# chhylp123/hifiasm

Measured on AMD Instinct MI355X. Metric: read-pair overlaps/sec (sum ol->length / (ha_pt_gen + all-reads h_ec_lchain pass)), higher is better.
Workload: dtype u64 hashing / int32 + f64 chain scores

## Files before the change

### hifiasm_amd/csrc/hao_chain.cuh

```cuda
#pragma once
#include "hao_common.cuh"
#include "hao_host.hpp"
#include "hao_query.cuh"

#define HAO_MCOPY_MAX 3

struct hao_chain_rec {
	uint32_t x_pos_s, x_pos_e, y_pos_s, y_pos_e; int32_t score; uint32_t n_hits, hit_rel, fc_rel, fc_len, strand;
	uint32_t src_rel, in_place;
};

#define HH_ID(h)     ((h).w0 & 0x7fffffffu)
#define HH_STRAND(h) ((h).w0 >> 31)
#define HH_SPAN(h)   ((int32_t)((h).cnt & 0xffu))
#define HH_WGT(h)    ((int32_t)((h).cnt >> 8))

struct hao_cpar { double pen_gap, pen_skip, bw; int64_t max_skip, max_iter, max_dis, xl, yl; };

__device__ __forceinline__ int64_t hao_ext_len(int64_t x_beg, int64_t x_end, int64_t xl, int64_t y_beg, int64_t y_end, int64_t yl)
{
	if (x_beg <= y_beg) x_beg = 0; else x_beg -= y_beg;
	int64_t xr = xl - x_end - 1, yr = yl - y_end - 1;
	if (xr <= yr) x_end = xl - 1; else x_end += yr;
	return x_end - x_beg + 1;
}

__device__ __forceinline__ int32_t hao_band(const hao_hit_t &ai, const hao_hit_t &aj, const hao_cpar &P)
{
	int64_t sf_s = aj.self_offset, sf_e = (int64_t)ai.self_offset + 1, ot_s = aj.offset, ot_e = (int64_t)ai.offset + 1;
	int64_t sf_r = P.xl - sf_e, ot_r = P.yl - ot_e;
	if (sf_s <= ot_s) sf_s = 0; else sf_s -= ot_s;
	if (sf_r <= ot_r) sf_e = P.xl; else sf_e += ot_r;
	return (int32_t)((double)(sf_e - sf_s) * P.bw);
}

__device__ __forceinline__ int32_t hao_pair_score(const hao_hit_t &ai, const hao_hit_t &aj, const hao_cpar &P, int64_t *dd_out)
{
	int32_t dq = (int32_t)((int64_t)ai.self_offset - (int64_t)aj.self_offset); if (dq <= 0) return INT32_MIN;
	int32_t dr = (int32_t)((int64_t)ai.offset - (int64_t)aj.offset); if (dr <= 0) return INT32_MIN;
	int32_t dd = dr > dq ? dr - dq : dq - dr;
	if (dd > 16 && dd > hao_band(ai, aj, P)) return INT32_MIN;
	int32_t dg = dr < dq ? dr : dq, span = HH_SPAN(ai), sc = span < dg ? span : dg, wgt = HH_WGT(ai);
	if (wgt != 1) sc = sc >= wgt ? (wgt == 2 ? sc >> 1 : sc / wgt) : 1;
	if (dd) {
		double lin = P.pen_gap * (double)dd; const double skip = P.pen_skip * (double)dg;
		if (!(dd < 4 && lin + skip < 1.0)) {
			const double ap = (double)sc * (((double)dd / (double)dg) / P.bw);
			if (dd < 4) lin = lin > ap ? ap : lin; else lin = lin < ap ? ap : lin;
			lin += skip;
			sc -= (int32_t)lin;
		}
	} else if (dg > span) {
		sc -= (int32_t)(0.0 + P.pen_skip * (double)dg);
	}
	if (dd_out) *dd_out = dd;
	return sc;
}

__device__ __forceinline__ void hao_region(hao_chain_rec &o, int64_t xl, int64_t yl, int64_t sc, const hao_hit_t &beg, const hao_hit_t &end)
{
	o.strand = HH_STRAND(beg);
	o.x_pos_s = beg.self_offset; o.y_pos_s = beg.offset; o.x_pos_e = end.self_offset; o.y_pos_e = end.offset;
	if (o.x_pos_s <= o.y_pos_s) { o.y_pos_s -= o.x_pos_s; o.x_pos_s = 0; } else { o.x_pos_s -= o.y_pos_s; o.y_pos_s = 0; }
	int64_t xr = xl - o.x_pos_e - 1, yr = yl - o.y_pos_e - 1;
	if (xr <= yr) { o.x_pos_e = (uint32_t)(xl - 1); o.y_pos_e += (uint32_t)xr; } else { o.y_pos_e = (uint32_t)(yl - 1); o.x_pos_e += (uint32_t)yr; }
	o.score = (int32_t)sc;
}

__device__ __forceinline__ uint64_t hao_fc_entry(uint32_t site, int32_t shift)
{ uint32_t lo = shift < 0 ? ((uint32_t)(-shift) << 1 | 1u) : (uint32_t)shift << 1; return (uint64_t)site << 32 | lo; }

template<class HitAt>
__device__ uint32_t hao_fake_cigar(uint64_t *fc, const hao_chain_rec &o, HitAt hit, int64_t n_hit)
{
	int64_t pdd = INT32_MAX; uint32_t n = 0;
	fc[n++] = hao_fc_entry(o.x_pos_s, 0);
	for (int64_t k = 0; k < n_hit; ++k) {
		const hao_hit_t h = hit(k);
		int64_t dq = (int64_t)h.self_offset - o.x_pos_s, dr = (int64_t)h.offset - o.y_pos_s, dd = dr - dq;
		if (dd != pdd) { pdd = dd; fc[n++] = hao_fc_entry(h.self_offset, (int32_t)pdd); }
	}
	uint64_t last = fc[n - 1]; int32_t lsh = (int32_t)((uint32_t)last >> 1); if (last & 1) lsh = -lsh;
	if ((int64_t)(int32_t)(last >> 32) != (int64_t)o.x_pos_e) fc[n++] = hao_fc_entry(o.x_pos_e, lsh);
	return n;
}

// ... 104 lines not shown
						hao_region(rec[n_u], P.xl, P.yl, sc + plus, a[ii[n_v - 1]], a[ii[n_v0]]);
						c_nv0[n_u] = (uint32_t)n_v0; c_ni[n_u] = (uint32_t)(n_v - n_v0); ++n_u;
					} else n_v = n_v0;
				} else n_v = n_v0;
			}
			for (k = 0, i = 0; k < n_u; ++k) {
				n_v0 = c_nv0[k]; ni = c_ni[k];
				rec[k].hit_rel = (uint32_t)i; rec[k].n_hits = (uint32_t)ni; rec[k].src_rel = (uint32_t)i; rec[k].in_place = 0;
				if (A.hcode) hao_code_chain_lane(A, gs, a, i, ni, [&](int64_t q_) { return (int64_t)ii[n_v0 + (ni - q_ - 1)]; });
				for (j = 0; j < ni; ++j, ++i) des[i] = a[ii[n_v0 + (ni - j - 1)]];
				rec[k].fc_rel = fcn; rec[k].fc_len = hao_fake_cigar(fcs + fcn, rec[k], [&](int64_t q_) { return a[ii[n_v0 + (ni - q_ - 1)]]; }, ni); fcn += rec[k].fc_len;
			}
			A.nch[g] = (uint32_t)n_u; A.nout[g] = (uint32_t)i;
			return;
		} else {
			msc += plus; i = msc_i; cL = 0;
			while (i >= 0) { t[cL++] = i; i = p[i]; }
		}
	}
	hao_region(rec[0], P.xl, P.yl, msc, a[t[cL - 1]], a[t[0]]);
	if (A.hcode) hao_code_chain_lane(A, gs, a, 0, cL, [&](int64_t q_) { return (int64_t)t[cL - q_ - 1]; });
	for (i = 0; i < cL; ++i) des[i] = a[t[cL - i - 1]];
	rec[0].hit_rel = 0; rec[0].n_hits = (uint32_t)cL; rec[0].src_rel = 0; rec[0].in_place = 0; rec[0].fc_rel = 0; rec[0].fc_len = hao_fake_cigar(fcs, rec[0], [&](int64_t q_) { return a[t[cL - q_ - 1]]; }, cL);
	A.nch[g] = 1; A.nout[g] = (uint32_t)cL;
}


template<class HitP, class I32P, class I64P>
__device__ void hao_chain_generic_core(const hao_chain_args &A, const uint64_t g, const uint64_t gs, HitP a, const int64_t a_n, const uint32_t xid, const uint32_t yid,
		const uint32_t xl, const uint32_t yl, I32P f, I32P ii, I32P p, I64P t)
{
	A.nch[g] = 0; A.nout[g] = 0;
	if (yid == xid || a_n <= 0) return;
	hao_cpar P; P.pen_gap = A.par.pen_gap; P.pen_skip = A.par.pen_skip; P.bw = A.par.bw; P.max_skip = A.par.max_skip; P.max_iter = A.par.max_iter; P.max_dis = A.par.max_dis;
	P.xl = xl; P.yl = yl;
	int64_t plus = 0, msc = INT32_MIN, msc_i = INT32_MIN, movl = INT32_MAX, si = 0, ei = a_n;
	{
		int64_t l = 0, k, z; bool sorted = true;
		for (k = 1; k <= a_n; ++k) {
			t[k - 1] = 0; ii[k - 1] = 0;
			if (k < a_n && HH_STRAND(a[k]) == HH_STRAND(a[l])) {
				if (a[k].self_offset <= a[k - 1].self_offset || a[k].offset <= a[k - 1].offset) sorted = false;
				continue;
			}
			if (sorted) {
				int64_t plus0 = 0, msc0 = INT32_MIN, msc_i0 = INT32_MIN, ddt = 0, sc, dd = 0;
				p[l] = -1; f[l] = HH_SPAN(a[l]);
				if (f[l] >= msc0) { msc0 = f[l]; msc_i0 = l; }
				if (f[l] < plus0) plus0 = f[l];
				for (z = l + 1; z < k; ++z) {
					int32_t s = hao_pair_score(a[z], a[z - 1], P, &dd);
					if (s == INT32_MIN) break;
					sc = (int64_t)s + f[z - 1];
					if (sc < HH_SPAN(a[z])) break;
					p[z] = (int32_t)(z - 1); f[z] = (int32_t)sc; ddt += dd;
					if (f[z] >= msc0) { msc0 = f[z]; msc_i0 = z; }
					if (f[z] < plus0) plus0 = f[z];
				}
				if (z >= k && msc_i0 == k - 1) {
					if (k - l >= 2 && ddt > 16 && ddt > hao_band(a[k - 1], a[l], P)) msc_i0 = INT32_MIN;
					if (msc_i0 == k - 1) {
						if (msc0 >= msc) {
							int64_t ov = hao_ext_len(a[msc_i0].self_offset, a[msc_i0].self_offset, P.xl, a[msc_i0].offset, a[msc_i0].offset, P.yl);
							if (msc0 > msc || ov < movl) { msc = msc0; msc_i = msc_i0; movl = ov; }
						}
						if (plus0 < plus) plus = plus0;
						if (ei > k) si = k; else ei = l;
// ... 63 lines not shown
			for (int k = 0; k < HAO_TINY_MAX; ++k) if ((uint32_t)k < e.n) l_a[k * 64 + threadIdx.x] = src[k];
		}
		const hao_lane_arr<int32_t> f{l_f + threadIdx.x}, ii{l_ii + threadIdx.x}, p{l_p + threadIdx.x}; const hao_lane_arr<int64_t> t{l_t + threadIdx.x};
		hao_chain_generic_core(A, e.g, e.start, hao_lane_hits{l_a + threadIdx.x}, (int64_t)e.n, (uint32_t)(A.rid_lo + e.r), e.yid, e.xl, e.yl, f, ii, p, t);
	}
}

__device__ __forceinline__ hao_hit_t hao_shfl_hit(const hao_hit_t &h, int src)
{ hao_hit_t o; o.w0 = hao_bcast(h.w0, src); o.offset = hao_bcast(h.offset, src); o.self_offset = hao_bcast(h.self_offset, src); o.cnt = hao_bcast(h.cnt, src); return o; }
__device__ __forceinline__ hao_hit_t hao_shfl_up_hit(const hao_hit_t &h)
{ hao_hit_t o; o.w0 = hao_wave_shr1(h.w0, h.w0); o.offset = hao_wave_shr1(h.offset, h.offset); o.self_offset = hao_wave_shr1(h.self_offset, h.self_offset); o.cnt = hao_wave_shr1(h.cnt, h.cnt); return o; }

__global__ __launch_bounds__(64) __attribute__((amdgpu_num_sgpr(96))) void chain_group_kernel(hao_chain_args A, const hao_gent *list, uint64_t n_list, uint32_t *slow, int cls)
{
	const uint64_t li = blockIdx.x;
	if (li >= n_list) return;
	const int lane = hao_lane();
	__shared__ uint64_t l_eb[2][64];
	uint64_t (*eb)[64] = l_eb; uint32_t ce0 = 0, ce1 = 0;
	const unsigned long long tq0 = A.dbg_qc ? wall_clock64() : 0;
	const hao_gent e = list[li];
	const uint64_t g = e.g, gs = e.start; const int32_t a_n = (int32_t)e.n;
	const hao_hit_t *a = A.hits + gs;
	const uint32_t xid = (uint32_t)(A.rid_lo + e.r), yid = e.yid;
	if (yid == xid || a_n <= 0) {
		if (A.hcode) for (int32_t i = lane; i < a_n; i += 64) A.hcode[gs + i] = 0x08;
		if (lane == 0) { A.nch[g] = 0; A.nout[g] = 0; }
		return;
	}
	hao_hit_t hn = a[lane < a_n ? lane : 0];
	const uint16_t *hqg = A.hcode ? A.hq + gs : nullptr; uint8_t *hcg = A.hcode ? A.hcode + gs : nullptr;
	uint32_t qn = hcg ? hqg[lane < a_n ? lane : 0] : 0u, carry_q = 0;
	const hao_hit_t first0 = hao_shfl_hit(hn, 0);
	hao_cpar P; P.pen_gap = A.par.pen_gap; P.pen_skip = A.par.pen_skip; P.bw = A.par.bw; P.max_skip = A.par.max_skip; P.max_iter = A.par.max_iter; P.max_dis = A.par.max_dis;
	P.xl = e.xl; P.yl = e.yl;
	const unsigned long long tq1 = A.dbg_qc ? wall_clock64() + (first0.w0 & 0) : 0;
	int32_t carry_f = 0; hao_hit_t carry_h = first0; carry_h.w0 ^= 0x80000000u;
	bool fail0 = false, fail1 = false, seen = false; int32_t maxf0 = INT32_MIN, maxf1 = INT32_MIN, flast0 = 0, flast1 = 0, k1 = 0, n_bnd = 0;
	uint32_t ddt0 = 0, ddt1 = 0;
	uint32_t last0_so = first0.self_offset, last0_of = first0.offset, last1_so = last0_so, last1_of = last0_of;
	unsigned long long first = 1ULL;
	const uint32_t ulane = (uint32_t)lane;
	for (int32_t t0 = 0; t0 < a_n; t0 += 64) {
		const int32_t left = a_n - t0; const bool act = lane < left;
		const unsigned long long actm = left >= 64 ? ~0ULL : (1ULL << left) - 1ULL;
		const hao_hit_t h = hn;
		const uint32_t q = qn;
		if (left > 64) {
			const uint32_t j = min(ulane, (uint32_t)(left - 65)); const hao_hit_t *an = a + (t0 + 64);
			hn = an[j]; if (hcg) qn = (hqg + (t0 + 64))[j];
		}
		hao_hit_t ph; ph.w0 = hao_wave_shr1(h.w0, carry_h.w0); ph.offset = hao_wave_shr1(h.offset, carry_h.offset); ph.self_offset = hao_wave_shr1(h.self_offset, carry_h.self_offset); ph.cnt = 0;
		const bool bnd = (int32_t)(h.w0 ^ ph.w0) < 0, st = act && bnd;
		const unsigned long long Mst = __ballot(bnd) & actm, Mbnd = Mst & ~first;
		unsigned long long Mb = 0; uint32_t bthr = 64; int B = 0;
		if (seen) { Mb = actm; bthr = 0; }
		else if (Mbnd) { B = __ffsll((long long)Mbnd) - 1; Mb = (~0ULL << B) & actm; bthr = (uint32_t)B; }
		const int b = ulane >= bthr;
		if (hcg) {
			const int32_t idx = t0 + lane;
			const uint32_t pq = hao_wave_shr1(q, carry_q);
			const int32_t dq = (int32_t)(q - pq), sh = (int32_t)((h.offset - ph.offset) - (h.self_offset - ph.self_offset));
			bool exc = false;
			if (A.exc_every) { uint32_t ii = (uint32_t)idx, ee = A.exc_every; HAO_OPAQUE_U32(ii); HAO_OPAQUE_U32(ee); exc = ii % ee == ee - 1; }
			const uint8_t code = st ? (uint8_t)0x08 : ((dq < 1 || dq > 15 || sh < -8 || sh > 7 || q == 65535u || exc) ? (uint8_t)0xff : (uint8_t)((dq - 1) << 4 | (sh + 8)));
			if (act) hcg[idx] = code;
			carry_q = hao_bcast(q, 63);
		}
		const int32_t span = HH_SPAN(h);
		const int32_t dq = (int32_t)(h.self_offset - ph.self_offset), dr = (int32_t)(h.offset - ph.offset);
		bool bad = dq <= 0 || dr <= 0;
		const int32_t dd = dr > dq ? dr - dq : dq - dr, dg = dr < dq ? dr : dq;
		if (!bad && dd > 16) { if (dd > hao_band(h, ph, P)) bad = true; }
		int32_t sc = span < dg ? span : dg;
		{	const int32_t wgt = HH_WGT(h);
			if (wgt != 1) sc = sc >= wgt ? (wgt == 2 ? sc >> 1 : sc / wgt) : 1; }
		if (dd) {
			double lin = P.pen_gap * (double)dd; const double skip = P.pen_skip * (double)dg;
			if (!(dd < 4 && lin + skip < 1.0)) {
				const double ap = (double)sc * (((double)dd / (double)dg) / P.bw);
				if (dd < 4) lin = lin > ap ? ap : lin; else lin = lin < ap ? ap : lin;
				lin += skip;
				sc -= (int32_t)lin;
			}
		} else if (dg > span) sc -= (int32_t)(0.0 + P.pen_skip * (double)dg);
		const bool scored = act && !bnd && !bad;
		const int32_t s = bad ? INT32_MIN : sc;
		const int32_t x = st ? span : (scored ? sc : 0);
		const uint32_t dde = scored ? (uint32_t)dd : 0u;
		{	const bool cf = act && (bnd || dr != dq);
			const unsigned long long Mcf = (__ballot(dr != dq) | Mst) & actm;
			const uint32_t n0 = (uint32_t)__popcll(Mcf & ~Mb), n1 = (uint32_t)__popcll(Mcf & Mb);
			if (cf) { const uint32_t at = hao_mbcnt(Mcf) + (b ? ce1 - n0 : ce0); if (at < 64) eb[b][at] = (uint64_t)h.self_offset << 32 | (h.offset - h.self_offset); }
			ce0 += n0; ce1 += n1; }
		const int32_t F = (int32_t)hao_wave_incl_scan_u32((uint32_t)x);
		int32_t f;
		if (Mbnd) {
			n_bnd += __popcll(Mbnd);
			const int32_t sub = B ? hao_bcast(F, B - 1) : 0;
			f = lane >= B ? F - sub : F + carry_f;
			if (B) { flast0 = hao_bcast(f, B - 1); last0_so = hao_bcast(h.self_offset, B - 1); last0_of = hao_bcast(h.offset, B - 1); }
			else { flast0 = carry_f; last0_so = carry_h.self_offset; last0_of = carry_h.offset; }
		} else f = F + carry_f;
		const int32_t fp = hao_wave_shr1(f, carry_f);
		const unsigned long long Mbrk = __ballot(hao_add_sat_i32(s, fp) < span) & actm & ~Mst;
		if (Mbrk & ~Mb) fail0 = true;
		if (Mbrk & Mb) fail1 = true;
		if (bthr == 64) { maxf0 = max(maxf0, f); ddt0 = hao_add_sat_u32(ddt0, dde); }
		else if (bthr == 0) { maxf1 = max(maxf1, f); ddt1 = hao_add_sat_u32(ddt1, dde); }
		else if (b == 0) { maxf0 = max(maxf0, f); ddt0 = hao_add_sat_u32(ddt0, dde); } else { maxf1 = max(maxf1, f); ddt1 = hao_add_sat_u32(ddt1, dde); }
		k1 += __popcll(actm & ~Mb);
		if (left <= 64) {
			const int Ls = left - 1; const int32_t vf = hao_bcast(f, Ls); const uint32_t vso = hao_bcast(h.self_offset, Ls), vof = hao_bcast(h.offset, Ls);
			if ((Mb >> Ls) & 1ULL) { flast1 = vf; last1_so = vso; last1_of = vof; } else { flast0 = vf; last0_so = vso; last0_of = vof; }
		}
		carry_f = hao_bcast(f, 63); carry_h = hao_shfl_hit(h, 63);
		if (Mbnd) seen = true;
		first = 0;
// ... 29 lines not shown
	hao_region(rc, P.xl, P.yl, msc, best ? first1 : first0, best ? last1 : last0);
	uint32_t cnt; const uint32_t ce = best ? ce1 : ce0;
	if (ce <= 64) {
		HAO_WAVE_FENCE();
		const int64_t cdiag = (int64_t)rc.y_pos_s - (int64_t)rc.x_pos_s;
		if (lane == 0) fcs[0] = hao_fc_entry(rc.x_pos_s, 0);
		if ((uint32_t)lane < ce) { const uint64_t raw = eb[best][lane]; fcs[1 + lane] = hao_fc_entry((uint32_t)(raw >> 32), (int32_t)((int64_t)(int32_t)(uint32_t)raw - cdiag)); }
		const uint64_t rlast = eb[best][ce - 1];
		cnt = 1 + ce;
		if ((uint32_t)(rlast >> 32) != rc.x_pos_e) { if (lane == 0) fcs[cnt] = hao_fc_entry(rc.x_pos_e, (int32_t)((int64_t)(int32_t)(uint32_t)rlast - cdiag)); ++cnt; }
	} else cnt = hao_fake_cigar_wave(fcs, rc.x_pos_s, rc.y_pos_s, rc.x_pos_e, cL, [&](int64_t k) { return a[bl + k]; });
	if (lane == 0) {
		rc.hit_rel = 0; rc.n_hits = (uint32_t)cL; rc.src_rel = (uint32_t)bl; rc.in_place = 1; rc.fc_rel = 0; rc.fc_len = cnt;
		A.rec[g * HAO_MCOPY_MAX] = rc; A.nch[g] = 1; A.nout[g] = (uint32_t)cL;
		if (A.dbg_qc && (li & 63) == 0) {  const unsigned long long tq3 = wall_clock64(); atomicAdd(A.dbg_qc, tq1 - tq0); atomicAdd(A.dbg_qc + 1, tq2 - tq1); atomicAdd(A.dbg_qc + 2, tq3 - tq2); atomicAdd(A.dbg_qc + 3, 1ULL); atomicAdd(A.dbg_qc + 4, (unsigned long long)a_n); }
	}
}


__global__ __launch_bounds__(256) void chain_pack8_kernel(hao_chain_args A, const hao_gent *list, uint64_t n_list, uint32_t *slow)
{
	const int lane = hao_lane(), wv = threadIdx.x >> 6, seg = lane >> 3, idx = lane & 7, sb = lane & ~7;
	const uint64_t li = ((uint64_t)blockIdx.x * 4 + wv) * 8 + seg;
	const bool have = li < n_list;
	hao_gent e; e.g = 0; e.r = 0; e.start = 0; e.n = 0; e.yid = 0; e.xl = 0; e.yl = 0;
	if (have) e = list[li];
	const int32_t a_n = (int32_t)e.n; const uint64_t g = e.g, gs = e.start;
	const uint32_t xid = (uint32_t)(A.rid_lo + e.r), yid = e.yid;
	const bool skip = !have || yid == xid || a_n <= 0;
	const bool act = !skip && idx < a_n;
	hao_hit_t h; h.w0 = 0; h.offset = 0; h.self_offset = 0; h.cnt = 0;
	if (act) h = A.hits[gs + idx];
	const uint32_t q = (A.hcode && act) ? A.hq[gs + idx] : 0u;
	hao_cpar P; P.pen_gap = A.par.pen_gap; P.pen_skip = A.par.pen_skip; P.bw = A.par.bw; P.max_skip = A.par.max_skip; P.max_iter = A.par.max_iter; P.max_dis = A.par.max_dis;
	P.xl = e.xl; P.yl = e.yl;
	const hao_hit_t ph = hao_shfl_up_hit(h);
	const uint32_t strand0 = (uint32_t)__shfl((int)HH_STRAND(h), sb);
	const bool st = act && (idx == 0 || HH_STRAND(h) != HH_STRAND(ph));
	const int b = act && HH_STRAND(h) != strand0;
	int32_t s = HH_SPAN(h); bool ok = true; int64_t dd = 0;
	if (act && !st) { s = hao_pair_score(h, ph, P, &dd); ok = s != INT32_MIN; if (!ok) { s = 0; dd = 0; } }
	uint8_t code = 0x08;
	if (A.hcode) {
		const uint32_t pq = hao_wave_shr1(q, 0u);
		const int32_t dq = (int32_t)(q - pq), sh = (int32_t)((h.offset - ph.offset) - (h.self_offset - ph.self_offset));
		if (!st) code = (dq < 1 || dq > 15 || sh < -8 || sh > 7 || q == 65535u || (A.exc_every && (uint32_t)idx % A.exc_every == A.exc_every - 1)) ? (uint8_t)0xff : (uint8_t)((dq - 1) << 4 | (sh + 8));
	}
	const uint32_t diag = h.offset - h.self_offset, pdiag = ph.offset - ph.self_offset;
	const bool cf = act && (st || diag != pdiag);
	int32_t x = act ? s : 0; int fl = (st || idx == 0) ? 1 : 0;
	hao_seg_scan_add(x, fl);
	const int32_t f = x, fp = hao_wave_shr1(f, 0);
	const bool brk = act && !st && (!ok || (int64_t)s + fp < (int64_t)HH_SPAN(h));
	auto seg_byte = [&](unsigned long long m) { return (uint32_t)(m >> sb) & 0xffu; };
	const uint32_t in0 = seg_byte(__ballot(act && b == 0)), brk0 = seg_byte(__ballot(brk && b == 0)), brk1 = seg_byte(__ballot(brk && b == 1)),
				   cf0 = seg_byte(__ballot(cf && b == 0)), cf1 = seg_byte(__ballot(cf && b == 1));
	const int32_t k1 = __popc(in0);
	const bool two = k1 < a_n;
	int32_t maxf0 = (act && b == 0) ? f : INT32_MIN, maxf1 = (act && b == 1) ? f : INT32_MIN, ddt0 = (act && b == 0) ? (int32_t)dd : 0, ddt1 = (act && b == 1) ? (int32_t)dd : 0;
#pragma unroll
	for (int d = 1; d < 8; d <<= 1) { maxf0 = max(maxf0, __shfl_xor(maxf0, d)); maxf1 = max(maxf1, __shfl_xor(maxf1, d)); ddt0 += __shfl_xor(ddt0, d); ddt1 += __shfl_xor(ddt1, d); }
	const int l0 = sb + (k1 > 0 ? k1 - 1 : 0), f1 = sb + (two ? k1 : 0), l1 = sb + (a_n > 0 ? a_n - 1 : 0);
	const int32_t flast0 = __shfl(f, l0), flast1 = __shfl(f, l1);
	hao_hit_t first0, last0, first1, last1;
	first0.w0 = (uint32_t)__shfl((int)h.w0, sb); first0.self_offset = (uint32_t)__shfl((int)h.self_offset, sb); first0.offset = (uint32_t)__shfl((int)h.offset, sb); first0.cnt = 0;
	last0.w0 = first0.w0; last0.self_offset = (uint32_t)__shfl((int)h.self_offset, l0); last0.offset = (uint32_t)__shfl((int)h.offset, l0); last0.cnt = 0;
	first1.w0 = (uint32_t)__shfl((int)h.w0, f1); first1.self_offset = (uint32_t)__shfl((int)h.self_offset, f1); first1.offset = (uint32_t)__shfl((int)h.offset, f1); first1.cnt = 0;
// ... 101 lines not shown
				}
				cn[6] = nu;
			}
			HAO_WAVE_FENCE();
			const uint32_t n_u = cn[6]; uint32_t o = 0, fcn = 0;
			for (uint32_t k = 0; k < n_u; ++k) {
				const int64_t n_v0 = cn[k], ni = cn[3 + k]; hao_chain_rec rc = l_rec[k];
				for (int64_t j = lane; j < ni; j += 64) des[o + j] = a[ii[n_v0 + (ni - j - 1)]];
				if (A.hcode) hao_code_chain_wave(A, gs, a, (int64_t)o, ni, [&](int64_t q_) { return (int64_t)ii[n_v0 + (ni - q_ - 1)]; });
				rc.hit_rel = o; rc.n_hits = (uint32_t)ni; rc.src_rel = o; rc.in_place = 0; rc.fc_rel = fcn;
				rc.fc_len = hao_fake_cigar_wave(fcs + fcn, rc.x_pos_s, rc.y_pos_s, rc.x_pos_e, ni, [&](int64_t q) { return a[ii[n_v0 + (ni - q - 1)]]; });
				fcn += rc.fc_len; o += (uint32_t)ni;
				if (lane == 0) rec[k] = rc;
			}
			if (lane == 0) { A.nch[g] = n_u; A.nout[g] = o; }
			return;
		}
		msc += plus; cL = 0;
		if (lane == 0) for (int64_t i = msc_i; i >= 0; i = p[i]) t[cL++] = i;
		cL = __shfl(cL, 0);
		HAO_WAVE_FENCE();
	}
	hao_chain_rec rc;
	hao_region(rc, P.xl, P.yl, msc, a[t[cL - 1]], a[t[0]]);
	for (int64_t i = lane; i < cL; i += 64) des[i] = a[t[cL - i - 1]];
	if (A.hcode) hao_code_chain_wave(A, gs, a, (int64_t)0, cL, [&](int64_t q_) { return (int64_t)t[cL - q_ - 1]; });
	rc.hit_rel = 0; rc.n_hits = (uint32_t)cL; rc.src_rel = 0; rc.in_place = 0; rc.fc_rel = 0;
	rc.fc_len = hao_fake_cigar_wave(fcs, rc.x_pos_s, rc.y_pos_s, rc.x_pos_e, cL, [&](int64_t q) { return a[t[cL - q - 1]]; });
	if (lane == 0) { rec[0] = rc; A.nch[g] = 1; A.nout[g] = (uint32_t)cL; }
}

#define HAO_DP_CAP 2048

template<int CAP, bool STAGE, bool INLDS>
__device__ __forceinline__ void hao_dp_body(const hao_chain_args &A, const hao_gent &e, const hao_hit_t *ag,
		int32_t *l_f, int32_t *l_p, int32_t *l_tm, int32_t *l_ii, int64_t *l_t, hao_hit_t *l_a, uint32_t *l_cn, hao_chain_rec *l_rec)
{
	const int lane = hao_lane();
	const uint64_t g = e.g, gs = e.start; const int64_t a_n = e.n;
	if (STAGE && INLDS) { for (int64_t i = lane; i < a_n; i += 64) l_a[i] = ag[i]; HAO_WAVE_FENCE(); }
	const hao_hit_t *a = (STAGE && INLDS) ? l_a : ag;
	hao_cpar P; P.pen_gap = A.par.pen_gap; P.pen_skip = A.par.pen_skip; P.bw = A.par.bw; P.max_skip = A.par.max_skip; P.max_iter = A.par.max_iter; P.max_dis = A.par.max_dis;
	P.xl = e.xl; P.yl = e.yl;
	int32_t *f = INLDS ? l_f : A.f + gs, *p = INLDS ? l_p : A.p + gs, *tm = INLDS ? l_tm : A.tm + gs;
	int32_t *ii = INLDS ? l_ii : A.ii + gs; int64_t *t = INLDS ? l_t : A.t + gs;
	const uint32_t strand0 = HH_STRAND(a[0]);
	int32_t carry_f = 0; hao_hit_t carry_h = a[0];
	bool fail0 = false, fail1 = false; int32_t maxf0 = INT32_MIN, maxf1 = INT32_MIN, flast0 = 0, flast1 = 0; int64_t ddt0 = 0, ddt1 = 0, k1 = 0;
	hao_hit_t last0 = a[0], last1 = a[0];
	for (int64_t t0 = 0; t0 < a_n; t0 += 64) {
		const int64_t idx = t0 + lane; const bool act = idx < a_n;
		hao_hit_t h = act ? a[idx] : carry_h;
		hao_hit_t ph = hao_shfl_up_hit(h); if (lane == 0) ph = carry_h;
		const bool st = act && (idx == 0 || HH_STRAND(h) != HH_STRAND(ph));
		const int b = act && HH_STRAND(h) != strand0;
		int32_t s = HH_SPAN(h); bool ok = true; int64_t dd = 0;
		if (act && !st) { s = hao_pair_score(h, ph, P, &dd); ok = s != INT32_MIN; if (!ok) { s = 0; dd = 0; } }
		int32_t x = act ? s : 0; int fl = st;
		hao_seg_scan_add(x, fl);
		if (!fl) x += carry_f;
		const int32_t fv = x; const int32_t fp = hao_wave_shr1(fv, carry_f);
		const bool brk = act && !st && (!ok || (int64_t)s + fp < (int64_t)HH_SPAN(h));
		if (__ballot(brk && b == 0)) fail0 = true;
		if (__ballot(brk && b == 1)) fail1 = true;
		if (act) { if (b == 0) { maxf0 = max(maxf0, fv); ddt0 += dd; } else { maxf1 = max(maxf1, fv); ddt1 += dd; } f[idx] = fv; p[idx] = st ? -1 : (int32_t)(idx - 1); tm[idx] = -1; ii[idx] = 0; t[idx] = 0; }
		k1 += __popcll(__ballot(act && b == 0));
		const bool isend = act && (idx == a_n - 1 || HH_STRAND(a[idx + 1]) != HH_STRAND(h));
		unsigned long long m0 = __ballot(isend && b == 0), m1 = __ballot(isend && b == 1);
		if (m0) { int src = __ffsll((long long)m0) - 1; flast0 = hao_bcast(fv, src); last0 = hao_shfl_hit(h, src); }
		if (m1) { int src = __ffsll((long long)m1) - 1; flast1 = hao_bcast(fv, src); last1 = hao_shfl_hit(h, src); }
		carry_f = hao_bcast(fv, 63); carry_h = hao_shfl_hit(h, 63);
	}
	maxf0 = hao_wave_max_i32(maxf0); maxf1 = hao_wave_max_i32(maxf1); ddt0 = hao_wave_sum_i64(ddt0); ddt1 = hao_wave_sum_i64(ddt1);
	const bool two = k1 < a_n;
	const hao_hit_t first0 = a[0], first1 = two ? a[k1] : a[0];
	const bool acc0 = !fail0 && flast0 == maxf0 && !(k1 >= 2 && ddt0 > 16 && ddt0 > hao_band(last0, first0, P));
	const bool acc1 = two && !fail1 && flast1 == maxf1 && !(a_n - k1 >= 2 && ddt1 > 16 && ddt1 > hao_band(last1, first1, P));
	int64_t plus = 0, msc = INT32_MIN, msc_i = INT32_MIN, movl = INT32_MAX, si = 0, ei = a_n;
	if (acc0) {
		msc = flast0; msc_i = k1 - 1; movl = hao_ext_len(last0.self_offset, last0.self_offset, P.xl, last0.offset, last0.offset, P.yl);
		if (ei > k1) si = k1; else ei = 0;
	}
	if (acc1) {
		if ((int64_t)flast1 >= msc) {
			int64_t ov = hao_ext_len(last1.self_offset, last1.self_offset, P.xl, last1.offset, last1.offset, P.yl);
			if ((int64_t)flast1 > msc || ov < movl) { msc = flast1; msc_i = a_n - 1; movl = ov; }
		}
		if (ei > a_n) si = a_n; else ei = k1;
	}
	__builtin_amdgcn_fence(__ATOMIC_RELEASE, "workgroup"); __builtin_amdgcn_fence(__ATOMIC_ACQUIRE, "workgroup");
	uint32_t n_spec_ok_out = 0, n_spec_fail_out = 0;
	{
		int64_t i, st, max_ii = -1; int spec_wait = 0, spec_fail = 0; uint32_t n_spec_ok = 0, n_spec_fail = 0;
		const bool spec_on = A.dbg_seq != 4;
		for (i = st = si; i < ei; ++i) {
			if (spec_wait > 0) --spec_wait;
			else if (spec_on) {
				int64_t st2 = st; if (i - st2 > P.max_iter) st2 = i - P.max_iter;
				const hao_hit_t h0 = a[i]; const uint32_t str_i = HH_STRAND(h0);
				while (str_i != HH_STRAND(a[st2])) ++st2;
				if (i == st2 || max_ii == i - 1) {
					const int64_t ti = i + lane; const bool inb = ti < ei;
					const hao_hit_t hi = inb ? a[ti] : h0;
					bool cand = inb && HH_STRAND(hi) == str_i && ti - st2 <= P.max_iter;
					int32_t s1 = 0;
					if (cand && ti > st2) {
						const hao_hit_t hp = a[ti - 1];
						s1 = hao_pair_score(hi, hp, P, nullptr);
						cand = s1 != INT32_MIN && s1 > 0 && (int64_t)hi.self_offset <= P.max_dis + (int64_t)hp.self_offset;
					}
					const unsigned long long badm = __ballot(!cand);
					const int nc = badm ? __ffsll((long long)badm) - 1 : 64;
					int64_t fg = ti > st2 ? (int64_t)s1 : (int64_t)HH_SPAN(hi);
					if (lane == 0 && i > st2) fg += f[i - 1];
					if (lane >= nc) fg = 0;
#pragma unroll
					for (int d = 1; d < 64; d <<= 1) { const int64_t y = __shfl_up(fg, d); if (lane >= d) fg += y; }
					const int32_t fg32 = (int32_t)fg; const int64_t pg = ti > st2 ? ti - 1 : -1;
					if (lane < nc) { f[ti] = fg32; p[ti] = (int32_t)pg; }
					HAO_WAVE_FENCE();
					int64_t mf = HH_SPAN(hi), mj = -1; int nsk = 0; unsigned long long marks = 0; bool done = lane >= nc;
					for (int d = 1; d <= 64; ++d) {
						const int64_t j = ti - d; const bool in = !done && j >= st2;
						if (!__ballot(in)) break;
						if (in) {
							const hao_hit_t hj = a[j]; const int32_t sj = hao_pair_score(hi, hj, P, nullptr);
							if (sj != INT32_MIN) {
								const int64_t sc = (int64_t)sj + f[j]; const int32_t pj = p[j];
								if (sc > mf) { mf = sc; mj = j; if (nsk > 0) --nsk; }
								else if (marks >> (d - 1) & 1) { if (++nsk > (int)P.max_skip) done = true; }
								if (pj >= 0) { const int64_t bb = ti - 1 - pj; if (bb < 64) marks |= 1ULL << bb; }
							}
						}
					}
					const bool ok = lane < nc && (done || ti - 65 < st2) && mf == (int64_t)fg32 && mj == pg;
					const unsigned long long nokm = __ballot(!ok);
					const int m = nokm ? __ffsll((long long)nokm) - 1 : 64;
					if (m > 0) {
						int32_t fmx = lane < m ? fg32 : INT32_MIN, fmn = lane < m ? fg32 : INT32_MAX;
#pragma unroll
						for (int d = 32; d >= 1; d >>= 1) { fmx = max(fmx, __shfl_xor(fmx, d)); fmn = min(fmn, __shfl_xor(fmn, d)); }
						if ((int64_t)fmx >= msc) {
							const int64_t ovl = hao_ext_len(hi.self_offset, hi.self_offset, P.xl, hi.offset, hi.offset, P.yl);
							int64_t key = (lane < m && fg32 == fmx) ? ovl * 64 + lane : INT64_MAX;
#pragma unroll
							for (int d = 32; d >= 1; d >>= 1) { const int64_t y = __shfl_xor(key, d); if (y < key) key = y; }
							if ((int64_t)fmx > msc || (key >> 6) < movl) { msc = fmx; msc_i = i + (key & 63); movl = key >> 6; }
						}
						if ((int64_t)fmn < plus) plus = fmn;
						max_ii = i + m - 1; st = st2; i += m - 1;
						if (m >= 8) spec_fail = 0;
						if (m < 64) spec_wait = 1;
						n_spec_ok += m;
						continue;
					}
					if (spec_fail < 5) ++spec_fail;
					spec_wait = 1 << spec_fail; ++n_spec_fail;
				}
			}
			const hao_hit_t hi = a[i];
			int64_t max_f = HH_SPAN(hi), n_skip = 0, max_j = -1, end_j;
			if (i - st > P.max_iter) st = i - P.max_iter;
			while (HH_STRAND(hi) != HH_STRAND(a[st])) ++st;
			end_j = st - 1;
			for (int64_t jb = i - 1; jb >= st; jb -= 64) {
				const int64_t j = jb - lane; const bool actv = j >= st;
				int32_t s = INT32_MIN; hao_hit_t hj; int32_t pj = -1; int64_t sc = INT64_MIN;
				if (actv) { hj = a[j]; s = hao_pair_score(hi, hj, P, nullptr); }
				const bool valid = actv && s != INT32_MIN;
				if (valid) { sc = (int64_t)s + f[j]; pj = p[j]; if (pj >= 0) tm[pj] = (int32_t)i; }
				__builtin_amdgcn_fence(__ATOMIC_RELEASE, "workgroup"); __builtin_amdgcn_fence(__ATOMIC_ACQUIRE, "workgroup");
				const bool mark = valid && tm[j] == (int32_t)i;
				const unsigned long long vm = __ballot(valid);
				unsigned long long imask = 0, rem = vm; int64_t cur = max_f;
				while (rem) {
					const unsigned long long gm = __ballot(valid && sc > cur) & rem;
					if (!gm) break;
					const int l = __ffsll((long long)gm) - 1;
					imask |= 1ULL << l; cur = hao_readlane_i64(sc, l); rem = l == 63 ? 0 : (vm & (~0ULL << (l + 1)));
				}
				const unsigned long long cmask = __ballot(mark) & ~imask;
				int brk_lane = -1; int64_t nsk = n_skip;
				if (cmask == 0 || imask == 0 || (63 - __clzll((long long)imask)) < (__ffsll((long long)cmask) - 1)) {
					nsk -= __popcll(imask); if (nsk < 0) nsk = 0;
					const int64_t need = P.max_skip + 1 - nsk;
					if ((int64_t)__popcll(cmask) >= need) brk_lane = __ffsll((long long)__ballot((cmask >> lane & 1) && (int64_t)__popcll(cmask & ((1ULL << lane) - 1)) == need - 1)) - 1;
					else nsk += __popcll(cmask);
				} else {
					unsigned long long ev = imask | cmask;
					while (ev) {
						const int l = __ffsll((long long)ev) - 1; ev &= ev - 1;
						if (imask >> l & 1) { if (nsk > 0) --nsk; } else if (++nsk > P.max_skip) { brk_lane = l; break; }
					}
				}
				n_skip = nsk;
				if (brk_lane >= 0) imask &= (1ULL << brk_lane) - 1;
				if (imask) { const int src = 63 - __clzll((long long)imask); max_f = hao_readlane_i64(sc, src); max_j = jb - src; }
				if (brk_lane >= 0) { end_j = jb - brk_lane; break; }
			}
			if (max_ii < 0 || (int64_t)hi.self_offset > (int64_t)a[max_ii].self_offset + P.max_dis || HH_STRAND(hi) != HH_STRAND(a[max_ii])) {
				int32_t mx = INT32_MIN; max_ii = -1;
				for (int64_t j = i - 1; j >= st && (int64_t)hi.self_offset <= P.max_dis + (int64_t)a[j].self_offset && HH_STRAND(hi) == HH_STRAND(a[j]); --j)
					if (mx < f[j]) { mx = f[j]; max_ii = j; }
			}
			if (max_ii >= 0 && max_ii < end_j && HH_STRAND(hi) == HH_STRAND(a[max_ii])) {
				int32_t tmp = hao_pair_score(hi, a[max_ii], P, nullptr);
				if (tmp != INT32_MIN && max_f < (int64_t)tmp + f[max_ii]) { max_f = (int64_t)tmp + f[max_ii]; max_j = max_ii; }
			}
			if (lane == 0) { f[i] = (int32_t)max_f; p[i] = (int32_t)max_j; }
			__builtin_amdgcn_fence(__ATOMIC_RELEASE, "workgroup"); __builtin_amdgcn_fence(__ATOMIC_ACQUIRE, "workgroup");
			if (max_ii < 0 || ((int64_t)hi.self_offset <= P.max_dis + (int64_t)a[max_ii].self_offset && HH_STRAND(hi) == HH_STRAND(a[max_ii]) && f[max_ii] < (int32_t)max_f)) max_ii = i;
			if ((int32_t)max_f >= msc) {
				int64_t ovl = hao_ext_len(hi.self_offset, hi.self_offset, P.xl, hi.offset, hi.offset, P.yl);
				if ((int32_t)max_f > msc || ovl < movl) { msc = (int32_t)max_f; msc_i = i; movl = ovl; }
			}
			if ((int32_t)max_f < plus) plus = (int32_t)max_f;
		}
		n_spec_ok_out = n_spec_ok; n_spec_fail_out = n_spec_fail;
	}
	if (A.dbg_stats && lane == 0) { atomicAdd(A.stats + HAO_NCLS + 1, (unsigned long long)n_spec_ok_out); atomicAdd(A.stats + HAO_NCLS + 2, (unsigned long long)n_spec_fail_out); atomicAdd(A.stats + HAO_NCLS + 3, (unsigned long long)(ei - si)); }
	if (A.dbg_seq == 3) { if (lane == 0) hao_chain_tail(A, g, a, a_n, P, f, p, t, ii, msc, msc_i, plus); return; }
	hao_chain_tail_wave(A, g, gs, a, a_n, P, f, p, t, ii, INLDS ? (int64_t)CAP : (int64_t)0, l_cn, l_rec, msc, msc_i, plus);
}

template<int CAP, bool STAGE>
__device__ __forceinline__ void hao_dp_kernel_body(const hao_chain_args &A, const hao_gent *list, const uint32_t *slow, const unsigned long long *slow_cnt)
{
	__shared__ int32_t l_f[CAP], l_p[CAP], l_tm[CAP], l_ii[CAP]; __shared__ int64_t l_t[CAP]; __shared__ hao_hit_t l_a[STAGE ? CAP : 1];
	__shared__ uint32_t l_cn[8]; __shared__ hao_chain_rec l_rec[HAO_MCOPY_MAX];
	const uint64_t n_slow = *slow_cnt;
	for (uint64_t b = blockIdx.x; b < n_slow; b += gridDim.x) {
		const hao_gent e = list[slow[b]];
		if (A.dbg_seq == 1) { if (hao_lane() == 0) hao_chain_generic(A, e.g); continue; }
		const hao_hit_t *ag = A.hits + e.start;
		if ((int64_t)e.n <= CAP) hao_dp_body<CAP, STAGE, true>(A, e, ag, l_f, l_p, l_tm, l_ii, l_t, l_a, l_cn, l_rec);
		else hao_dp_body<CAP, STAGE, false>(A, e, ag, l_f, l_p, l_tm, l_ii, l_t, l_a, l_cn, l_rec);
		HAO_WAVE_FENCE();
	}
}

template<int CAP, bool STAGE>
__global__ __launch_bounds__(64) void chain_dp_kernel(hao_chain_args A, const hao_gent *list, const uint32_t *slow, const unsigned long long *slow_cnt)
{ hao_dp_kernel_body<CAP, STAGE>(A, list, slow, slow_cnt); }
__global__ __launch_bounds__(64) __attribute__((amdgpu_waves_per_eu(4, 8))) void chain_dp128_kernel(hao_chain_args A, const hao_gent *list, const uint32_t *slow, const unsigned long long *slow_cnt)
{ hao_dp_kernel_body<128, true>(A, list, slow, slow_cnt); }

struct hao_cdesc {
	uint64_t src;
	uint64_t dst;
	uint32_t n, w0;
	uint32_t r, pad;
};
#define HAO_CD_OHITS (1ULL << 63)
__device__ __forceinline__ const hao_hit_t *hao_cd_src(const hao_cdesc &d, const hao_hit_t *hits, const hao_hit_t *ohits)
{ return ((d.src & HAO_CD_OHITS) ? ohits : hits) + (d.src & ~HAO_CD_OHITS); }

struct hao_asm_args {
	const uint64_t *g_start; const uint32_t *g_read; const uint8_t *g_cls; const uint64_t *g_off; uint64_t n_groups; uint64_t rid_lo;
	const hao_hit_t *ohits, *hits; const uint64_t *fcs; const hao_chain_rec *rec; const uint32_t *nch;
	const uint64_t *ch_base, *cl_base, *fc_base;
	hao_ovlp_t *ol; uint64_t *ol_fc_off; hao_cdesc *cd; uint64_t *fc;
};

__global__ __launch_bounds__(256) void chain_assemble_kernel(hao_asm_args A)
{
	const uint64_t g = (uint64_t)blockIdx.x * 256 + threadIdx.x; const int lane = hao_lane();
	const uint32_t n = g < A.n_groups ? A.nch[g] : 0;
	uint32_t r = 0; uint64_t ord0 = 0, cl0 = 0, gs = 0, chb = 0, clb = 0; uint32_t yid = 0;
	if (n) {
		r = A.g_read[g]; const uint64_t g0 = A.g_off[r];
		chb = A.ch_base[g]; clb = A.cl_base[g]; ord0 = chb - A.ch_base[g0]; cl0 = A.cl_base[g0]; gs = A.g_start[g];
		yid = HH_ID(A.hits[gs]);
	}
#pragma unroll
	for (uint32_t c = 0; c < HAO_MCOPY_MAX; ++c) {
		const bool has = c < n; uint32_t fl = 0; uint64_t fd = 0; const uint64_t *fs = nullptr;
		if (has) {
			const hao_chain_rec rc = A.rec[g * HAO_MCOPY_MAX + c];
// ... 767 lines not shown
```

### hifiasm_amd/csrc/hao_host.hpp

```cpp
#pragma once
#include <cmath>
#include <cstdint>
#include <vector>
#include "hao.h"

static int hao_adjust_to_prior(int prior, int top, int left, int right, int *peak_het)
{
	const int64_t cand[3] = { left, top, right };
	int best = -1; int64_t best_d = -1;
	for (int i = 0; i < 3; ++i) {
		if (cand[i] <= 0) continue;
		const int64_t d = cand[i] >= prior ? cand[i] - prior : prior - cand[i];
		if (best_d == -1 || d < best_d || (d == best_d && i == 1)) { best_d = d; best = i; }
	}
	if (best < 0) return prior;
	if (cand[best] < prior && (double)(prior - cand[best]) >= cand[best] * 0.51) { *peak_het = (int)cand[best]; return prior; }
	for (int i = best - 1; i >= 0; --i) if (cand[i] > 0) { *peak_het = (int)cand[i]; break; }
	return (int)cand[best];
}

static int hao_find_peaks(const int64_t *cnt, int n_cnt, int start_cnt, int *peak_het, int prior_hom = -1)
{
	*peak_het = -1;
	const int first = cnt[1] > 0 ? 1 : 2;
// ... 17 lines not shown
		if (right_v < top_v * 0.05 || min_between(top + 1, right) > right_v * 0.95 || right > top * 2.5) right = -1;
	}
	if (prior_hom > 0) return hao_adjust_to_prior(prior_hom, top, left, right, peak_het);
	if (right > 0) { *peak_het = top; return right; }
	if (left > 0) *peak_het = left;
	return top;
}

static inline void hao_occ_thresholds(int hom_cov, uint32_t *high_occ, uint32_t *low_occ)
{
	*high_occ = (uint32_t)(hom_cov * (2.0 - 0.333));
	*low_occ = (uint32_t)(hom_cov * 0.333);
}

static inline void hao_seed_weight_table(uint32_t high_occ, uint32_t low_occ, std::vector<uint32_t> &tab)
{
	const uint64_t hi = high_occ < 2 ? 2 : high_occ, lo = low_occ < 2 ? 2 : low_occ;
	tab.resize(4096);
	for (uint64_t n = 0; n < 4096; ++n) {
		uint32_t wgt;
		if (n < hi && n > lo) wgt = 1;
		else if (n <= lo) wgt = 2;
		else { wgt = (uint32_t)(1 + ((n + (hi << 1) - 1) / (hi << 1))); wgt = (uint32_t)pow((double)wgt, 1.1); }
		if (wgt > 0xffffffu) wgt = 0xffffffu;
		tab[n] = wgt;
	}
}

struct hao_chain_par {
	double pen_gap, pen_skip, bw;
	int64_t max_skip, max_iter, max_dis;
	int64_t mcopy_num; double mcopy_rate; int64_t mcopy_khit_cut;
	uint32_t chain_cutoff; uint64_t ocv_w; uint64_t max_n_chain;
};

static inline hao_chain_par hao_chain_params(int k, const hao_pass_t &ps)
{
	hao_chain_par p;
	double tmp = expf(-0.01 * (double)k);
	p.pen_gap = 0.5f * tmp; p.pen_skip = 0.0005f * tmp;
	p.max_skip = 25; p.max_iter = 5000; p.max_dis = 5000;
	p.bw = ps.bw_thres;
	p.mcopy_num = ps.mcopy_num; p.mcopy_rate = ps.mcopy_rate; p.mcopy_khit_cut = ps.mcopy_khit_cut; p.chain_cutoff = ps.chain_cutoff; p.ocv_w = ps.ocv_w;
	p.max_n_chain = (uint64_t)ps.max_n_chain;
	return p;
}
```

Before: 179.6 million.

## Skip fp64 gap penalty via host-precomputed integer thresholds in chain scoring

Precomputes on the host, for each small diagonal difference, the gap length below which the fp64 penalty rounds to zero, and packs these limits into a 64-bit word. Device pair scoring checks this integer threshold and takes the double-precision penalty path only when it can change the score. In the wave-scan kernel the check is made wave-uniform with ballots, and parameters are pinned in registers. The 128-cap DP kernel keeps the unconditional path. The risk is exactness if the host threshold search does not match device floating-point rounding.

```diff
diff --git a/hifiasm_amd/csrc/hao_chain.cuh b/hifiasm_amd/csrc/hao_chain.cuh
--- a/hifiasm_amd/csrc/hao_chain.cuh
+++ b/hifiasm_amd/csrc/hao_chain.cuh
@@ -15,7 +15,13 @@
 #define HH_SPAN(h)   ((int32_t)((h).cnt & 0xffu))
 #define HH_WGT(h)    ((int32_t)((h).cnt >> 8))
 
-struct hao_cpar { double pen_gap, pen_skip, bw; int64_t max_skip, max_iter, max_dis, xl, yl; };
+struct hao_cpar { double pen_gap, pen_skip, bw; int64_t max_skip, max_iter, max_dis, xl, yl; uint64_t lim16; };
+__device__ __forceinline__ hao_cpar hao_cpar_of(const hao_chain_par &par)
+{
+	hao_cpar P; P.pen_gap = par.pen_gap; P.pen_skip = par.pen_skip; P.bw = par.bw; P.max_skip = par.max_skip; P.max_iter = par.max_iter; P.max_dis = par.max_dis; P.xl = P.yl = 0;
+	P.lim16 = par.lim16;
+	return P;
+}
 
 __device__ __forceinline__ int64_t hao_ext_len(int64_t x_beg, int64_t x_end, int64_t xl, int64_t y_beg, int64_t y_end, int64_t yl)
 {
@@ -34,6 +40,17 @@
 	return (int32_t)((double)(sf_e - sf_s) * P.bw);
 }
 
+__device__ __forceinline__ uint64_t hao_vreg_u64(uint64_t x) { uint32_t lo = (uint32_t)x, hi = (uint32_t)(x >> 32); HAO_OPAQUE_U32(lo); HAO_OPAQUE_U32(hi); return (uint64_t)hi << 32 | lo; }
+__device__ __forceinline__ double hao_vreg_f64(double x) { union { double d; uint64_t u; } c; c.d = x; c.u = hao_vreg_u64(c.u); return c.d; }
+
+__device__ __forceinline__ int32_t hao_pen_lim(int32_t dd, uint64_t lim16) { return (int32_t)((uint32_t)(lim16 >> (((uint32_t)dd << 4) & 63u)) & 0xffffu); }
+__device__ __forceinline__ bool hao_pen_fp64(int32_t dd, int32_t dg, int32_t span, uint64_t lim16)
+{
+	const int32_t lim = hao_pen_lim(dd, lim16);
+	return (bool)((int)(dd > 3) | ((int)(dg >= lim) & ((int)(dd != 0) | (int)(dg > span))));
+}
+
+template<bool THR = true>
 __device__ __forceinline__ int32_t hao_pair_score(const hao_hit_t &ai, const hao_hit_t &aj, const hao_cpar &P, int64_t *dd_out)
 {
 	int32_t dq = (int32_t)((int64_t)ai.self_offset - (int64_t)aj.self_offset); if (dq <= 0) return INT32_MIN;
@@ -42,16 +59,18 @@
 	if (dd > 16 && dd > hao_band(ai, aj, P)) return INT32_MIN;
 	int32_t dg = dr < dq ? dr : dq, span = HH_SPAN(ai), sc = span < dg ? span : dg, wgt = HH_WGT(ai);
 	if (wgt != 1) sc = sc >= wgt ? (wgt == 2 ? sc >> 1 : sc / wgt) : 1;
-	if (dd) {
-		double lin = P.pen_gap * (double)dd; const double skip = P.pen_skip * (double)dg;
-		if (!(dd < 4 && lin + skip < 1.0)) {
-			const double ap = (double)sc * (((double)dd / (double)dg) / P.bw);
-			if (dd < 4) lin = lin > ap ? ap : lin; else lin = lin < ap ? ap : lin;
-			lin += skip;
-			sc -= (int32_t)lin;
-		}
-	} else if (dg > span) {
-		sc -= (int32_t)(0.0 + P.pen_skip * (double)dg);
+	if (!THR || hao_pen_fp64(dd, dg, span, P.lim16)) {
+		if (dd) {
+			double lin = P.pen_gap * (double)dd; const double skip = P.pen_skip * (double)dg;
+			if (!(dd < 4 && lin + skip < 1.0)) {
+				const double ap = (double)sc * (((double)dd / (double)dg) / P.bw);
+				if (dd < 4) lin = lin > ap ? ap : lin; else lin = lin < ap ? ap : lin;
+				lin += skip;
+				sc -= (int32_t)lin;
+			}
+		} else if (dg > span) {
+			sc -= (int32_t)(0.0 + P.pen_skip * (double)dg);
+		}
 	}
 	if (dd_out) *dd_out = dd;
 	return sc;
@@ -222,7 +241,7 @@
 {
 	A.nch[g] = 0; A.nout[g] = 0;
 	if (yid == xid || a_n <= 0) return;
-	hao_cpar P; P.pen_gap = A.par.pen_gap; P.pen_skip = A.par.pen_skip; P.bw = A.par.bw; P.max_skip = A.par.max_skip; P.max_iter = A.par.max_iter; P.max_dis = A.par.max_dis;
+	hao_cpar P = hao_cpar_of(A.par);
 	P.xl = xl; P.yl = yl;
 	int64_t plus = 0, msc = INT32_MIN, msc_i = INT32_MIN, movl = INT32_MAX, si = 0, ei = a_n;
 	{
@@ -352,7 +371,7 @@
 	const uint16_t *hqg = A.hcode ? A.hq + gs : nullptr; uint8_t *hcg = A.hcode ? A.hcode + gs : nullptr;
 	uint32_t qn = hcg ? hqg[lane < a_n ? lane : 0] : 0u, carry_q = 0;
 	const hao_hit_t first0 = hao_shfl_hit(hn, 0);
-	hao_cpar P; P.pen_gap = A.par.pen_gap; P.pen_skip = A.par.pen_skip; P.bw = A.par.bw; P.max_skip = A.par.max_skip; P.max_iter = A.par.max_iter; P.max_dis = A.par.max_dis;
+	hao_cpar P = hao_cpar_of(A.par);
 	P.xl = e.xl; P.yl = e.yl;
 	const unsigned long long tq1 = A.dbg_qc ? wall_clock64() + (first0.w0 & 0) : 0;
 	int32_t carry_f = 0; hao_hit_t carry_h = first0; carry_h.w0 ^= 0x80000000u;
@@ -361,6 +380,8 @@
 	uint32_t last0_so = first0.self_offset, last0_of = first0.offset, last1_so = last0_so, last1_of = last0_of;
 	unsigned long long first = 1ULL;
 	const uint32_t ulane = (uint32_t)lane;
+	const uint64_t lim16 = hao_vreg_u64(P.lim16);
+	P.pen_gap = hao_vreg_f64(P.pen_gap); P.pen_skip = hao_vreg_f64(P.pen_skip); P.bw = hao_vreg_f64(P.bw);
 	for (int32_t t0 = 0; t0 < a_n; t0 += 64) {
 		const int32_t left = a_n - t0; const bool act = lane < left;
 		const unsigned long long actm = left >= 64 ? ~0ULL : (1ULL << left) - 1ULL;
@@ -395,15 +416,18 @@
 		int32_t sc = span < dg ? span : dg;
 		{	const int32_t wgt = HH_WGT(h);
 			if (wgt != 1) sc = sc >= wgt ? (wgt == 2 ? sc >> 1 : sc / wgt) : 1; }
-		if (dd) {
-			double lin = P.pen_gap * (double)dd; const double skip = P.pen_skip * (double)dg;
-			if (!(dd < 4 && lin + skip < 1.0)) {
-				const double ap = (double)sc * (((double)dd / (double)dg) / P.bw);
-				if (dd < 4) lin = lin > ap ? ap : lin; else lin = lin < ap ? ap : lin;
-				lin += skip;
-				sc -= (int32_t)lin;
-			}
-		} else if (dg > span) sc -= (int32_t)(0.0 + P.pen_skip * (double)dg);
+		const int32_t lim = hao_pen_lim(dd, lim16);
+		if (__ballot(dd > 3) | (__ballot(dg >= lim) & (__ballot(dr != dq) | __ballot(dg > span)))) {
+			if (dd) {
+				double lin = P.pen_gap * (double)dd; const double skip = P.pen_skip * (double)dg;
+				if (!(dd < 4 && lin + skip < 1.0)) {
+					const double ap = (double)sc * (((double)dd / (double)dg) / P.bw);
+					if (dd < 4) lin = lin > ap ? ap : lin; else lin = lin < ap ? ap : lin;
+					lin += skip;
+					sc -= (int32_t)lin;
+				}
+			} else if (dg > span) sc -= (int32_t)(0.0 + P.pen_skip * (double)dg);
+		}
 		const bool scored = act && !bnd && !bad;
 		const int32_t s = bad ? INT32_MIN : sc;
 		const int32_t x = st ? span : (scored ? sc : 0);
@@ -499,7 +523,7 @@
 	hao_hit_t h; h.w0 = 0; h.offset = 0; h.self_offset = 0; h.cnt = 0;
 	if (act) h = A.hits[gs + idx];
 	const uint32_t q = (A.hcode && act) ? A.hq[gs + idx] : 0u;
-	hao_cpar P; P.pen_gap = A.par.pen_gap; P.pen_skip = A.par.pen_skip; P.bw = A.par.bw; P.max_skip = A.par.max_skip; P.max_iter = A.par.max_iter; P.max_dis = A.par.max_dis;
+	hao_cpar P = hao_cpar_of(A.par);
 	P.xl = e.xl; P.yl = e.yl;
 	const hao_hit_t ph = hao_shfl_up_hit(h);
 	const uint32_t strand0 = (uint32_t)__shfl((int)HH_STRAND(h), sb);
@@ -667,7 +691,7 @@
 
 #define HAO_DP_CAP 2048
 
-template<int CAP, bool STAGE, bool INLDS>
+template<int CAP, bool STAGE, bool INLDS, bool THR>
 __device__ __forceinline__ void hao_dp_body(const hao_chain_args &A, const hao_gent &e, const hao_hit_t *ag,
 		int32_t *l_f, int32_t *l_p, int32_t *l_tm, int32_t *l_ii, int64_t *l_t, hao_hit_t *l_a, uint32_t *l_cn, hao_chain_rec *l_rec)
 {
@@ -675,7 +699,7 @@
 	const uint64_t g = e.g, gs = e.start; const int64_t a_n = e.n;
 	if (STAGE && INLDS) { for (int64_t i = lane; i < a_n; i += 64) l_a[i] = ag[i]; HAO_WAVE_FENCE(); }
 	const hao_hit_t *a = (STAGE && INLDS) ? l_a : ag;
-	hao_cpar P; P.pen_gap = A.par.pen_gap; P.pen_skip = A.par.pen_skip; P.bw = A.par.bw; P.max_skip = A.par.max_skip; P.max_iter = A.par.max_iter; P.max_dis = A.par.max_dis;
+	hao_cpar P = hao_cpar_of(A.par);
 	P.xl = e.xl; P.yl = e.yl;
 	int32_t *f = INLDS ? l_f : A.f + gs, *p = INLDS ? l_p : A.p + gs, *tm = INLDS ? l_tm : A.tm + gs;
 	int32_t *ii = INLDS ? l_ii : A.ii + gs; int64_t *t = INLDS ? l_t : A.t + gs;
@@ -690,7 +714,7 @@
 		const bool st = act && (idx == 0 || HH_STRAND(h) != HH_STRAND(ph));
 		const int b = act && HH_STRAND(h) != strand0;
 		int32_t s = HH_SPAN(h); bool ok = true; int64_t dd = 0;
-		if (act && !st) { s = hao_pair_score(h, ph, P, &dd); ok = s != INT32_MIN; if (!ok) { s = 0; dd = 0; } }
+		if (act && !st) { s = hao_pair_score<THR>(h, ph, P, &dd); ok = s != INT32_MIN; if (!ok) { s = 0; dd = 0; } }
 		int32_t x = act ? s : 0; int fl = st;
 		hao_seg_scan_add(x, fl);
 		if (!fl) x += carry_f;
@@ -741,7 +765,7 @@
 					int32_t s1 = 0;
 					if (cand && ti > st2) {
 						const hao_hit_t hp = a[ti - 1];
-						s1 = hao_pair_score(hi, hp, P, nullptr);
+						s1 = hao_pair_score<THR>(hi, hp, P, nullptr);
 						cand = s1 != INT32_MIN && s1 > 0 && (int64_t)hi.self_offset <= P.max_dis + (int64_t)hp.self_offset;
 					}
 					const unsigned long long badm = __ballot(!cand);
@@ -759,7 +783,7 @@
 						const int64_t j = ti - d; const bool in = !done && j >= st2;
 						if (!__ballot(in)) break;
 						if (in) {
-							const hao_hit_t hj = a[j]; const int32_t sj = hao_pair_score(hi, hj, P, nullptr);
+							const hao_hit_t hj = a[j]; const int32_t sj = hao_pair_score<THR>(hi, hj, P, nullptr);
 							if (sj != INT32_MIN) {
 								const int64_t sc = (int64_t)sj + f[j]; const int32_t pj = p[j];
 								if (sc > mf) { mf = sc; mj = j; if (nsk > 0) --nsk; }
@@ -801,7 +825,7 @@
 			for (int64_t jb = i - 1; jb >= st; jb -= 64) {
 				const int64_t j = jb - lane; const bool actv = j >= st;
 				int32_t s = INT32_MIN; hao_hit_t hj; int32_t pj = -1; int64_t sc = INT64_MIN;
-				if (actv) { hj = a[j]; s = hao_pair_score(hi, hj, P, nullptr); }
+				if (actv) { hj = a[j]; s = hao_pair_score<THR>(hi, hj, P, nullptr); }
 				const bool valid = actv && s != INT32_MIN;
 				if (valid) { sc = (int64_t)s + f[j]; pj = p[j]; if (pj >= 0) tm[pj] = (int32_t)i; }
 				__builtin_amdgcn_fence(__ATOMIC_RELEASE, "workgroup"); __builtin_amdgcn_fence(__ATOMIC_ACQUIRE, "workgroup");
@@ -839,7 +863,7 @@
 					if (mx < f[j]) { mx = f[j]; max_ii = j; }
 			}
 			if (max_ii >= 0 && max_ii < end_j && HH_STRAND(hi) == HH_STRAND(a[max_ii])) {
-				int32_t tmp = hao_pair_score(hi, a[max_ii], P, nullptr);
+				int32_t tmp = hao_pair_score<THR>(hi, a[max_ii], P, nullptr);
 				if (tmp != INT32_MIN && max_f < (int64_t)tmp + f[max_ii]) { max_f = (int64_t)tmp + f[max_ii]; max_j = max_ii; }
 			}
 			if (lane == 0) { f[i] = (int32_t)max_f; p[i] = (int32_t)max_j; }
@@ -858,7 +882,7 @@
 	hao_chain_tail_wave(A, g, gs, a, a_n, P, f, p, t, ii, INLDS ? (int64_t)CAP : (int64_t)0, l_cn, l_rec, msc, msc_i, plus);
 }
 
-template<int CAP, bool STAGE>
+template<int CAP, bool STAGE, bool THR = true>
 __device__ __forceinline__ void hao_dp_kernel_body(const hao_chain_args &A, const hao_gent *list, const uint32_t *slow, const unsigned long long *slow_cnt)
 {
 	__shared__ int32_t l_f[CAP], l_p[CAP], l_tm[CAP], l_ii[CAP]; __shared__ int64_t l_t[CAP]; __shared__ hao_hit_t l_a[STAGE ? CAP : 1];
@@ -868,8 +892,8 @@
 		const hao_gent e = list[slow[b]];
 		if (A.dbg_seq == 1) { if (hao_lane() == 0) hao_chain_generic(A, e.g); continue; }
 		const hao_hit_t *ag = A.hits + e.start;
-		if ((int64_t)e.n <= CAP) hao_dp_body<CAP, STAGE, true>(A, e, ag, l_f, l_p, l_tm, l_ii, l_t, l_a, l_cn, l_rec);
-		else hao_dp_body<CAP, STAGE, false>(A, e, ag, l_f, l_p, l_tm, l_ii, l_t, l_a, l_cn, l_rec);
+		if ((int64_t)e.n <= CAP) hao_dp_body<CAP, STAGE, true, THR>(A, e, ag, l_f, l_p, l_tm, l_ii, l_t, l_a, l_cn, l_rec);
+		else hao_dp_body<CAP, STAGE, false, THR>(A, e, ag, l_f, l_p, l_tm, l_ii, l_t, l_a, l_cn, l_rec);
 		HAO_WAVE_FENCE();
 	}
 }
@@ -878,7 +902,7 @@
 __global__ __launch_bounds__(64) void chain_dp_kernel(hao_chain_args A, const hao_gent *list, const uint32_t *slow, const unsigned long long *slow_cnt)
 { hao_dp_kernel_body<CAP, STAGE>(A, list, slow, slow_cnt); }
 __global__ __launch_bounds__(64) __attribute__((amdgpu_waves_per_eu(4, 8))) void chain_dp128_kernel(hao_chain_args A, const hao_gent *list, const uint32_t *slow, const unsigned long long *slow_cnt)
-{ hao_dp_kernel_body<128, true>(A, list, slow, slow_cnt); }
+{ hao_dp_kernel_body<128, true, false>(A, list, slow, slow_cnt); }
 
 struct hao_cdesc {
 	uint64_t src;
diff --git a/hifiasm_amd/csrc/hao_host.hpp b/hifiasm_amd/csrc/hao_host.hpp
--- a/hifiasm_amd/csrc/hao_host.hpp
+++ b/hifiasm_amd/csrc/hao_host.hpp
@@ -73,13 +73,36 @@
 	int64_t max_skip, max_iter, max_dis;
 	int64_t mcopy_num; double mcopy_rate; int64_t mcopy_khit_cut;
 	uint32_t chain_cutoff; uint64_t ocv_w; uint64_t max_n_chain;
+	uint64_t lim16; int32_t dg_lim[4], skip0_lim;
 };
+
+template<class Pred>
+static inline int32_t hao_first_dg(Pred fails)
+{
+	if (fails(1)) return 1;
+	int32_t lo = 1, hi = INT32_MAX;
+	while (hi - lo > 1) { const int32_t mid = lo + (hi - lo) / 2; if (fails(mid)) hi = mid; else lo = mid; }
+	return hi;
+}
+static inline void hao_penalty_thresholds(hao_chain_par &p)
+{
+#if defined(__clang__)
+#pragma clang fp contract(off)
+#endif
+	p.dg_lim[0] = 0;
+	for (int32_t dd = 1; dd < 4; ++dd)
+		p.dg_lim[dd] = hao_first_dg([&](int32_t dg) { double lin = p.pen_gap * (double)dd; const double skip = p.pen_skip * (double)dg; return !(lin + skip < 1.0); });
+	p.skip0_lim = hao_first_dg([&](int32_t dg) { const double v = 0.0 + p.pen_skip * (double)dg; return v >= 2147483648.0 || (int32_t)v >= 1; });
+	auto s16 = [](int32_t v) { return (uint64_t)(v > 65535 ? 65535 : v); };
+	p.lim16 = s16(p.skip0_lim) | s16(p.dg_lim[1]) << 16 | s16(p.dg_lim[2]) << 32 | s16(p.dg_lim[3]) << 48;
+}
 
 static inline hao_chain_par hao_chain_params(int k, const hao_pass_t &ps)
 {
 	hao_chain_par p;
 	double tmp = expf(-0.01 * (double)k);
 	p.pen_gap = 0.5f * tmp; p.pen_skip = 0.0005f * tmp;
+	hao_penalty_thresholds(p);
 	p.max_skip = 25; p.max_iter = 5000; p.max_dis = 5000;
 	p.bw = ps.bw_thres;
 	p.mcopy_num = ps.mcopy_num; p.mcopy_rate = ps.mcopy_rate; p.mcopy_khit_cut = ps.mcopy_khit_cut; p.chain_cutoff = ps.chain_cutoff; p.ocv_w = ps.ocv_w;
```

After: 180.8 million (median of 3 runs). Within noise of the previous version (+0.6%).
